# PSeitz/veloci

Measured on AMD Instinct MI355X. Metric: queries/sec, 3-term AND on 100M-doc index (p50 latency and HBM fraction alongside), higher is better.
Workload: dtype u32 doc ids + f16->f32 scores

## Files before the change

veloci_amd/csrc/scan_probe.hip:

```cpp
#include <hip/hip_runtime.h>
#include <hip/hip_fp16.h>

#include "device_types.hpp"
#include "kernel_common.hpp"
#include "kernels.hpp"
#include "probe_common.hpp"

namespace vq {

#ifdef VQ_STAMP
__device__ unsigned long long g_probe_stamp[16];
#define PS_INIT                                                      \
    unsigned long long _st0 = __builtin_amdgcn_s_memtime();          \
    const unsigned long long _t0 = _st0;                             \
    const unsigned long long _r0 = __builtin_amdgcn_s_memrealtime(); \
    unsigned long long _acc[16] = {0};
#define PS_AT(k)                                                \
    {                                                           \
        unsigned long long _st1 = __builtin_amdgcn_s_memtime(); \
        _acc[k] += _st1 - _st0;                                 \
        _st0 = _st1;                                            \
    }
#define PS_COUNT(k) _acc[k] += 1ull;
#define PS_FLUSH                                                                                             \
    _acc[14] = __builtin_amdgcn_s_memtime() - _t0;                        \
    _acc[15] = __builtin_amdgcn_s_memrealtime() - _r0;                \
    if (threadIdx.x == 0) {                                                                                  \
        _Pragma("unroll") for (int _k = 0; _k < 16; ++_k) if (_acc[_k]) atomicAdd(&g_probe_stamp[_k], _acc[_k]); \
    }
void debug_read_probe_stamps(unsigned long long* out, int reset) {
    (void)hipMemcpyFromSymbol(out, HIP_SYMBOL(g_probe_stamp), sizeof(unsigned long long) * 16);
    if (reset) {
        unsigned long long z[16] = {0};
        (void)hipMemcpyToSymbol(HIP_SYMBOL(g_probe_stamp), z, sizeof z);
    }
}
#else
#define PS_INIT
#define PS_AT(k)
#define PS_COUNT(k)
#define PS_FLUSH
#endif

constexpr uint32_t kPMaxR = 2;
constexpr uint32_t kPU = 256;
static_assert(kPU >= 256, "a round of 256 postings must fit the empty queue");
constexpr uint32_t kPR = 128;
constexpr uint32_t kPLdsShape = 8;
constexpr uint32_t kPLdsU = kPLdsShape + 24;
constexpr uint32_t kPLdsR = kPLdsU + kPU;
__host__ __device__ constexpr uint32_t probe_lds_tile(uint32_t nd) { return kPLdsR + (2 + nd) * kPR; }
__host__ __device__ constexpr uint32_t probe_lds_arr(uint32_t nd, uint32_t nb) { return probe_lds_tile(nd) + nb * (kPTW + kPRk); }
size_t scan_probe_lds_bytes(uint32_t cand_cap, uint32_t nd, uint32_t na, uint32_t arr_slot) {
    return (size_t)(probe_lds_arr(nd, nd - na) + na * arr_slot + 2 * cand_cap) * 4 + 16;
}

template <uint32_t ND, uint32_t NA, bool OR = false>
__device__ __forceinline__ void probe_body(const uint8_t* __restrict__ blob, const uint32_t span, const uint32_t q, const uint32_t cand_cap, const uint32_t arr_slot,
                                           unsigned long long* __restrict__ span_keys, unsigned long long* __restrict__ num_hits) {
    extern __shared__ __attribute__((aligned(16))) uint32_t lds[];
    const uint32_t lane = threadIdx.x;
    const VQ_CONST QHeader* H = as_const<QHeader>(blob);
    const VQ_CONST DList* gl = as_const<DList>(blob + H->off_lists);
    const VQ_CONST DOp* gops = as_const<DOp>(blob + H->off_ops);
    const VQ_CONST DProbe* P = as_const<DProbe>(blob + H->off_simple2);
    const uint32_t sflags = H->simple_flags;
    const uint32_t top_k = H->top_k;
    constexpr uint32_t n = ND + 1u;
    constexpr uint32_t NB = ND - NA;
    constexpr uint32_t NB1 = NB ? NB : 1u, NA1 = NA ? NA : 1u;
    PS_INIT

    unsigned long long* thr = reinterpret_cast<unsigned long long*>(lds);
    uint32_t* cand_n = lds + 2;
    uint32_t* sh = lds + kPLdsShape;
    uint32_t* uq = lds + kPLdsU;
    uint32_t* rq = lds + kPLdsR;
    uint32_t* tile = lds + probe_lds_tile(ND);
    uint32_t* rank = tile + NB * kPTW;
    uint32_t* arr = lds + probe_lds_arr(ND, NB);
    unsigned long long* cand = reinterpret_cast<unsigned long long*>(arr + NA * arr_slot);
    unsigned long long* const gthr = reinterpret_cast<unsigned long long*>(const_cast<uint8_t*>(blob) + offsetof(QHeader, gthr));
    CandState cs{cand, cand_n, thr, cand_cap, gthr};
    cs.upper = H->key_upper;
    uint32_t* const stat = H->stat_off ? lds + 4 : nullptr;
    uint8_t* const pool = H->off_pool ? const_cast<uint8_t*>(blob) + H->off_pool : nullptr;

    const uint32_t* ccov = nullptr;
    const uint32_t* cgdir = nullptr;
    const uint32_t* d_bitmap[NB1];
    const uint32_t* d_rank[NB1];
    const uint16_t* d_arr[NA1];
    const uint32_t* d_agd[NA1];
    {
        const uint32_t ck = (uint32_t)__ffs((int)sf_cover_mask(sflags)) - 1u;
        const uint32_t am = sf_array_mask(sflags);
        uint32_t role_of[4] = {0u, 0u, 0u, 0u};
        uint32_t ib = 0, ia = NB;
#pragma unroll
        for (uint32_t k = 0; k < n; ++k) {
            const VQ_CONST DList& d = gl[gops[k].list_begin];
            if (k == ck) {
                ccov = P->leaf[k].cov32;
                cgdir = P->leaf[k].gdir;
                if (lane == 0) {
                    sh[kShCts] = __float_as_uint(d.term_score);
                    sh[kShPrunable] = (d.term_score > 0.0f && d.max_raw < 0x7C00u) ? 1u : 0u;
                }
            } else {
                const bool is_arr = ((am >> k) & 1u) != 0u;
                const uint32_t role = is_arr ? ia : ib;
#pragma unroll
                for (uint32_t j = 0; j < NB; ++j)
                    if (!is_arr && j == role) {
                        d_bitmap[j] = d.bitmap;
                        d_rank[j] = d.rank_dir;
                    }
#pragma unroll
                for (uint32_t a = 0; a < NA; ++a)
                    if (is_arr && NB + a == role) {
                        d_arr[a] = P->leaf[k].arr16;
                        d_agd[a] = P->leaf[k].gdir;
                    }
                if (lane == 0) {
                    const uint16_t mr = d.max_raw;
                    sh[kShTs + role] = __float_as_uint(d.term_score);
                    sh[kShVmax + role] = (d.term_score > 0.0f && mr < 0x7C00u) ? __float_as_uint(posting_value(d.term_score, mr)) : 0x7F800000u;
                    reinterpret_cast<unsigned long long*>(sh + kShScores)[role] = is_arr ? (unsigned long long)(uintptr_t)P->leaf[k].cov32 : (unsigned long long)(uintptr_t)d.scores;
                }
                role_of[k] = 1u + role;
                if (is_arr) ++ia;
                else ++ib;
            }
        }
        const KOp root(gops + n);
#pragma unroll
        for (uint32_t j = 0; j < n; ++j) {
            const uint32_t k = OR ? j : root.and_order(j);
            if (lane == 0) sh[kShSrc + j] = k == 0u ? role_of[0] : k == 1u ? role_of[1] : k == 2u ? role_of[2] : role_of[3];
        }
    }

    const uint32_t n_spans = H->n_spans;
    const unsigned long long range = (unsigned long long)(H->doc_hi - H->doc_lo);
    const uint32_t span_lo = span == 0 ? H->doc_lo : ((H->doc_lo + (uint32_t)(range * span / n_spans)) & ~(kPT - 1u));
    const uint32_t span_hi = span + 1 == n_spans ? H->doc_hi : ((H->doc_lo + (uint32_t)(range * (span + 1) / n_spans)) & ~(kPT - 1u));
    const uint32_t bitmap_base = H->bitmap_base;
    const uint32_t keys_base = H->keys_base;

    if (lane == 0) {
        *thr = __hip_atomic_load(gthr, __ATOMIC_RELAXED, __HIP_MEMORY_SCOPE_AGENT);
        *cand_n = 0;
        lds[4] = 0u;
    }
    __syncthreads();
    unsigned long long thr_seen = *thr;
    uint32_t raw_min = 0u;
    constexpr uint32_t kMasks = OR ? (1u << ND) : 1u;
    uint32_t rmin[kMasks];
    auto take_raw_min = [&](const float thr_f) {
        if (OR) {
#pragma unroll
            for (uint32_t m = 0; m < kMasks; ++m) rmin[m] = probe_raw_min<ND>(sh, thr_f, lane, m);
        } else raw_min = probe_raw_min<ND>(sh, thr_f, lane);
    };
    take_raw_min(__uint_as_float(unorder_f32((uint32_t)(thr_seen >> 32))));

    const u32x4 kSent = u32x4{0xFFFFFFFFu, 0xFFFFFFFFu, 0xFFFFFFFFu, 0xFFFFFFFFu};
    const VQ_GLOBAL u32x4* cc4 = as_global(reinterpret_cast<const u32x4*>(ccov));

    uint32_t un = 0, rn = 0;
    uint32_t ucnt = 0;
    unsigned long long hits = 0;
    unsigned long long g_prev = 0ull;

    const uint32_t t_first = (span_lo - bitmap_base) >> kProbeTileShift;
    const uint32_t t_end = span_hi > span_lo ? ((span_hi - 1u - bitmap_base) >> kProbeTileShift) + 1u : t_first;
    uint32_t dir_base = t_first;
    auto load_dir = [&](const uint32_t* g) { return as_global(g)[dir_base + lane < t_end ? dir_base + lane : t_end]; };
    uint32_t dirv = load_dir(cgdir);
    uint32_t adv[NA1];
#pragma unroll
    for (uint32_t a = 0; a < NA; ++a) adv[a] = load_dir(d_agd[a]);
    auto dir_at = [&](const uint32_t v, const uint32_t tt) { return (uint32_t)__builtin_amdgcn_readlane((int)v, (int)(tt - dir_base)); };

    u32x4 wk[ND][kPNV];
    uint32_t rk[NB1];
    u32x4 nid[kPMaxR], cid[kPMaxR];
#pragma unroll
    for (uint32_t r = 0; r < kPMaxR; ++r) nid[r] = cid[r] = kSent;
    uint32_t pf_rounds = 0, pf_v0 = 0, pf_v1 = 0;
    uint32_t na_g0[NA1], na_nv[NA1];
    uint32_t a_g0[NA1], a_cnt[NA1];
#pragma unroll
    for (uint32_t a = 0; a < NA1; ++a) na_g0[a] = na_nv[a] = a_g0[a] = a_cnt[a] = 0u;
    auto issue_tile = [&](const uint32_t tt, const uint32_t g0, const uint32_t g1) {
        pf_rounds = (g1 - g0 + 31u) >> 5;
        pf_v0 = g0 * 2u;
        pf_v1 = g1 * 2u;
        if (OR || pf_rounds) {
#pragma unroll
            for (uint32_t i = 0; i < NB; ++i) {
                const VQ_GLOBAL u32x4* gb = as_global(reinterpret_cast<const u32x4*>(d_bitmap[i] + (size_t)tt * kPTW));
#pragma unroll
                for (uint32_t h = 0; h < kPNV; ++h) wk[i][h] = gb[h * 64u + lane];
                rk[i] = as_global(d_rank[i])[tt * kPRk + lane];
            }
#pragma unroll
            for (uint32_t a = 0; a < NA; ++a) {
                const VQ_GLOBAL u32x4* ga = as_global(reinterpret_cast<const u32x4*>(d_arr[a]) + na_g0[a]);
#pragma unroll
                for (uint32_t h = 0; h < kPNV; ++h)
                    if (h * 64u + lane < na_nv[a]) wk[NB + a][h] = ga[h * 64u + lane];
            }
#pragma unroll
            for (uint32_t r = 0; r < kPMaxR; ++r) {
                const uint32_t v = pf_v0 + r * 64u + lane;
                nid[r] = kSent;
                if (r < pf_rounds && v < pf_v1) nid[r] = cc4[v];
            }
        }
    };

    uint32_t tile_lo = 0;
    uint32_t f_stage = 0;
    uint32_t f_doc = 0, f_idx[ND];
    float f_vc = 0.0f, f_vd[ND];
    uint16_t f_r = 0;
    bool f_alive = false;
#pragma unroll
    for (uint32_t i = 0; i < ND; ++i) {
        f_idx[i] = 0u;
        f_vd[i] = 0.0f;
    }
    uint32_t rhead = 0;
    uint32_t tiles_since_merge = 8;
    auto push_keys = [&](const unsigned long long key, bool pending, const bool final) {
        if (wballot(pending)) {
            while (true) {
                if (pending) {
                    if (key > *thr) {
                        uint32_t pos = atomicAdd(cs.n, 1u);
                        if (pos < cs.cap) {
                            cs.cand[pos] = key;
                            pending = false;
                        }
                    } else pending = false;
                }
                probe_lds_fence();
                if (!wballot(pending)) break;
                cand_prune(cs, top_k);
            }
            if (pool && (tiles_since_merge >= 8u || final)) {
                PS_COUNT(13)
                tiles_since_merge = 0;
                probe_pool_merge<true>(cs, top_k, pool, lane);
            }
            const unsigned long long tn = *thr;
            if ((uint32_t)(tn >> 32) != (uint32_t)(thr_seen >> 32)) take_raw_min(__uint_as_float(unorder_f32((uint32_t)(tn >> 32))));
            thr_seen = tn;
        }
    };
    uint32_t f_mask = 0;
    auto sum_of = [&](const ProbeShape<ND>& S, const float vc, const float (&vd)[ND], const uint32_t mask) { return OR ? probe_or_sum<ND>(S, vc, vd, mask) : probe_sum<ND>(S, vc, vd); };
    auto flush_final = [&](const ProbeShape<ND>& S, const bool final) {
        const float score = sum_of(S, f_vc, f_vd, f_mask);
        const unsigned long long key = ((unsigned long long)order_f32(__float_as_uint(score)) << 32) | (unsigned long long)f_doc;
        f_stage = 0;
        PS_COUNT(12)
        push_keys(key, f_alive && key > *thr && key < cs.upper, final);
    };
    auto flush_service = [&](const bool final) {
        const unsigned long long* sptr = reinterpret_cast<const unsigned long long*>(sh + kShScores);
        unsigned long long gp = sptr[0];
        uint32_t gidx = 0u;
        if (f_stage) {
            const ProbeShape<ND> S = probe_shape<ND>(sh);
            const float thr_f = __uint_as_float(unorder_f32((uint32_t)(*thr >> 32)));
            bool last = true;
#pragma unroll
            for (uint32_t i = 0; i < ND; ++i)
                if (f_stage == i + 1u) {
                    f_vd[i] = posting_value(S.ts[i], f_r);
                    if (i + 1u < ND) {
                        constexpr uint32_t zero = 0;
                        f_alive = f_alive && !(sum_of(S, f_vc, f_vd, f_mask) < thr_f);
                        if (stat && lane == 0) *stat += 2u * (uint32_t)__popcll(wballot(f_alive));
                        gp = sptr[i + 1u < ND ? i + 1u : zero];
                        gidx = (f_alive && (!OR || ((f_mask >> (i + 1u < ND ? i + 1u : zero)) & 1u))) ? f_idx[i + 1u < ND ? i + 1u : zero] : 0u;
                        last = false;
                    }
                }
            if (last) flush_final(S, final);
            else ++f_stage;
        } else if (rn >= 64u || (final && rn)) {
            const uint32_t count = rn < 64u ? rn : 64u;
            probe_lds_fence();
            f_alive = lane < count;
            uint32_t raw = 0;
            const uint32_t slot = (rhead + lane) & (kPR - 1u);
            if (f_alive) {
                f_doc = rq[slot];
                raw = rq[kPR + slot];
#pragma unroll
                for (uint32_t i = 0; i < ND; ++i) f_idx[i] = rq[(2u + i) * kPR + slot];
            }
            if (OR) {
                f_mask = 0u;
#pragma unroll
                for (uint32_t i = 0; i < ND; ++i) f_mask |= f_idx[i] != 0xFFFFFFFFu ? 1u << i : 0u;
            }
            f_vc = posting_value(__uint_as_float(sh[kShCts]), (uint16_t)raw);
#pragma unroll
            for (uint32_t i = 0; i < ND; ++i) f_vd[i] = __uint_as_float(sh[kShVmax + i]);
            if (stat && lane == 0) *stat += 2u * count;
            gidx = (f_alive && (!OR || (f_mask & 1u))) ? f_idx[0] : 0u;
            f_stage = 1u;
            rhead = (rhead + count) & (kPR - 1u);
            rn -= count;
        }
        f_r = as_global(reinterpret_cast<const uint16_t*>((uintptr_t)gp))[gidx];
    };
    auto flush_sync = [&]() {
        const ProbeShape<ND> S = probe_shape<ND>(sh);
        probe_lds_fence();
        const uint32_t slot = (rhead + lane) & (kPR - 1u);
        const uint32_t doc = rq[slot];
        const float vc = posting_value(S.cts, (uint16_t)rq[kPR + slot]);
        float vd[ND];
        uint32_t mask = 0;
#pragma unroll
        for (uint32_t i = 0; i < ND; ++i) {
            const uint16_t* sp = reinterpret_cast<const uint16_t*>((uintptr_t) reinterpret_cast<const unsigned long long*>(sh + kShScores)[i]);
            const uint32_t ix = rq[(2u + i) * kPR + slot];
            if (ix != 0xFFFFFFFFu) mask |= 1u << i;
            vd[i] = posting_value(S.ts[i], as_global(sp)[(OR && ix == 0xFFFFFFFFu) ? 0u : ix]);
        }
        if (stat && lane == 0) *stat += 2u * ND * 64u;
        const float score = sum_of(S, vc, vd, mask);
        const unsigned long long key = ((unsigned long long)order_f32(__float_as_uint(score)) << 32) | (unsigned long long)doc;
        rhead = (rhead + 64u) & (kPR - 1u);
        rn -= 64u;
        push_keys(key, key > *thr && key < cs.upper, false);
    };
    auto bitmap_rank = [&](const uint32_t i, const uint32_t rel) {
        const uint32_t g = rel >> kRankShift, wi = (rel >> 5) & 15u, below = (1u << (rel & 31u)) - 1u;
        const int full = (int)((1u << wi) - 1u);
        const uint32_t* tl = tile + i * kPTW;
        uint32_t acc = rank[i * kPRk + g] + (uint32_t)__popc(tl[rel >> 5] & below);
        const u32x4* gw = reinterpret_cast<const u32x4*>(tl + g * 16u);
#pragma unroll
        for (uint32_t v4 = 0; v4 < 4; ++v4) {
            const u32x4 x = gw[v4];
            acc += (uint32_t)__popc(x.x & (uint32_t)__builtin_amdgcn_sbfe(full, v4 * 4u + 0u, 1u));
            acc += (uint32_t)__popc(x.y & (uint32_t)__builtin_amdgcn_sbfe(full, v4 * 4u + 1u, 1u));
            acc += (uint32_t)__popc(x.z & (uint32_t)__builtin_amdgcn_sbfe(full, v4 * 4u + 2u, 1u));
            acc += (uint32_t)__popc(x.w & (uint32_t)__builtin_amdgcn_sbfe(full, v4 * 4u + 3u, 1u));
        }
        return acc;
    };
    auto rank_some = [&](const uint32_t cnt) {
        while (rn + cnt > kPR) flush_sync();
        probe_lds_fence();
        const uint32_t* const uqe = uq + (un - cnt);
        un -= cnt;
        if (NA == 0u && ND == 2u && cnt <= 32u) {
            const uint32_t el = lane & 31u, role = lane >> 5;
            if (el < cnt) {
                const uint32_t e = uqe[el];
                const uint32_t rel = e >> 16;
                const uint32_t slot = (rhead + rn + el) & (kPR - 1u);
                if (role == 0u) {
                    rq[slot] = tile_lo + rel;
                    rq[kPR + slot] = e & 0xFFFFu;
                }
                const bool here = !OR || ((tile[role * kPTW + (rel >> 5)] >> (rel & 31u)) & 1u) != 0u;
                rq[(2u + role) * kPR + slot] = here ? bitmap_rank(role, rel) : 0xFFFFFFFFu;
            }
            rn += cnt;
        } else if (NA == 0u) {
            if (lane < cnt) {
                const uint32_t e = uqe[lane];
                const uint32_t rel = e >> 16;
                const uint32_t slot = (rhead + rn + lane) & (kPR - 1u);
                rq[slot] = tile_lo + rel;
                rq[kPR + slot] = e & 0xFFFFu;
#pragma unroll
                for (uint32_t i = 0; i < NB; ++i) {
                    const bool here = !OR || ((tile[i * kPTW + (rel >> 5)] >> (rel & 31u)) & 1u) != 0u;
                    rq[(2u + i) * kPR + slot] = here ? bitmap_rank(i, rel) : 0xFFFFFFFFu;
                }
            }
            rn += cnt;
        } else {
            uint32_t e = 0xFFFFFFFFu, pos[NA1];
            bool found = lane < cnt;
            if (found) e = uqe[lane];
            const uint32_t rel = e >> 16;
#pragma unroll
            for (uint32_t a = 0; a < NA; ++a) {
                const uint16_t* A = reinterpret_cast<const uint16_t*>(arr + a * arr_slot);
                uint32_t lo = 0u, len = a_cnt[a];
#ifdef VQ_PROBE_NO_SEARCH
                lo = rel & 7u;
                len = 0u;
#endif
                while (len > 1u) {
                    const uint32_t half = len >> 1;
                    lo = (uint32_t)A[lo + half] <= rel ? lo + half : lo;
                    len -= half;
                }
#ifdef VQ_PROBE_NO_SEARCH
                found = found && a_cnt[a] != 0u && ((uint32_t)A[lo] ^ rel) < 0x2000u;
#else
                found = found && a_cnt[a] != 0u && (uint32_t)A[lo] == rel;
#endif
                pos[a] = lo;
            }
            const unsigned long long fm = wballot(found);
            hits += (unsigned long long)__popcll(fm);
            const bool live = found && (e & 0xFFFFu) >= raw_min;
            const unsigned long long lm = wballot(live);
            if (lm) {
                if (live) {
                    const uint32_t slot = (rhead + rn + (uint32_t)__popcll(lm & ((1ull << lane) - 1ull))) & (kPR - 1u);
                    rq[slot] = tile_lo + rel;
                    rq[kPR + slot] = e & 0xFFFFu;
#pragma unroll
                    for (uint32_t i = 0; i < NB; ++i) rq[(2u + i) * kPR + slot] = bitmap_rank(i, rel);
#pragma unroll
                    for (uint32_t a = 0; a < NA; ++a) rq[(2u + NB + a) * kPR + slot] = (a_g0[a] * 8u + pos[a]) * 2u;
                }
                rn += (uint32_t)__popcll(lm);
            }
        }
    };
    uint32_t lo_rel = 0, width = 0;
    struct ProbeWords {
        uint32_t w[OR ? ND : 1u][4];
    };
    auto probe_read = [&](const u32x4 e4) {
        const uint32_t ee[4] = {e4.x, e4.y, e4.z, e4.w};
        ProbeWords pw;
#pragma unroll
        for (uint32_t c = 0; c < 4; ++c) {
            const uint32_t a = (ee[c] >> 21) & (kPTW - 1u);
            if (OR) {
#pragma unroll
                for (uint32_t i = 0; i < ND; ++i) pw.w[OR ? i : 0u][c] = tile[i * kPTW + a];
            } else {
                pw.w[0][c] = 0xFFFFFFFFu;
                if (NB) {
                    pw.w[0][c] = tile[a];
#pragma unroll
                    for (uint32_t i = 1; i < NB; ++i) pw.w[0][c] &= tile[i * kPTW + a];
                }
            }
        }
        return pw;
    };
    auto probe_eval = [&](const u32x4 e4, const ProbeWords& pw, const bool may_overflow) {
        const uint32_t ee[4] = {e4.x, e4.y, e4.z, e4.w};
        unsigned long long lm[4];
        bool live[4];
#pragma unroll
        for (uint32_t c = 0; c < 4; ++c) {
            const uint32_t rel = ee[c] >> 16;
            const bool in = (rel - lo_rel) < width;
            if (OR) {
                uint32_t mask = 0;
#pragma unroll
                for (uint32_t i = 0; i < ND; ++i) mask |= ((pw.w[OR ? i : 0u][c] >> (rel & 31u)) & 1u) << i;
                uint32_t need = rmin[0];
#pragma unroll
                for (uint32_t m = 1; m < kMasks; ++m) need = mask == m ? rmin[OR ? m : 0u] : need;
                hits += (unsigned long long)__popcll(wballot(in && mask == 0u));
                live[c] = in && (ee[c] & 0xFFFFu) >= need;
                lm[c] = wballot(live[c]);
                continue;
            }
            const bool bit = ((pw.w[0][c] >> (rel & 31u)) & 1u) != 0u;
            const unsigned long long sm = NB ? (wballot(in) & wballot(bit)) : wballot(in);
            if (NA == 0u) {
                const bool strong = (ee[c] & 0xFFFFu) >= raw_min;
                hits += (unsigned long long)__popcll(sm);
                lm[c] = sm & wballot(strong);
                live[c] = in && bit && strong;
            } else {
                lm[c] = sm;
                live[c] = in && bit;
            }
        }
        if (lm[0] | lm[1] | lm[2] | lm[3]) {
            if (may_overflow) {
                const uint32_t add = (uint32_t)__popcll(lm[0]) + (uint32_t)__popcll(lm[1]) + (uint32_t)__popcll(lm[2]) + (uint32_t)__popcll(lm[3]);
                while (un + add > kPU) rank_some(un < 64u ? un : 64u);
            }
#pragma unroll
            for (uint32_t c = 0; c < 4; ++c) {
                if (live[c]) uq[un + (uint32_t)__popcll(lm[c] & ((1ull << lane) - 1ull))] = ee[c];
                un += (uint32_t)__popcll(lm[c]);
            }
        }
    };

    uint32_t t = t_first;
    tile_lo = bitmap_base + (t_first << kProbeTileShift);
    auto next_arrays = [&](const uint32_t tt) {
#pragma unroll
        for (uint32_t a = 0; a < NA; ++a) {
            na_g0[a] = dir_at(adv[a], tt);
            na_nv[a] = dir_at(adv[a], tt + 1u) - na_g0[a];
        }
    };
    if (t < t_end) {
        next_arrays(t);
        issue_tile(t, dir_at(dirv, t), dir_at(dirv, t + 1u));
    }
    PS_AT(0)
    while (t < t_end) {
        PS_COUNT(8)
        __builtin_amdgcn_s_waitcnt(0x0F70);
        __builtin_amdgcn_s_setprio(3);
        const uint32_t rounds = pf_rounds, v0 = pf_v0, v1 = pf_v1;
        if (OR || rounds) {
            if (OR) {
#pragma unroll
                for (uint32_t h = 0; h < kPNV; ++h) {
                    u32x4 u = wk[0][h];
#pragma unroll
                    for (uint32_t i = 1; i < NB; ++i) u |= wk[i][h];
                    ucnt += (uint32_t)__popc(u.x) + (uint32_t)__popc(u.y) + (uint32_t)__popc(u.z) + (uint32_t)__popc(u.w);
                }
            }
#pragma unroll
            for (uint32_t i = 0; i < NB; ++i) {
#pragma unroll
                for (uint32_t h = 0; h < kPNV; ++h) reinterpret_cast<u32x4*>(tile + i * kPTW)[h * 64u + lane] = wk[i][h];
                rank[i * kPRk + lane] = rk[i];
            }
#pragma unroll
            for (uint32_t a = 0; a < NA; ++a) {
#pragma unroll
                for (uint32_t h = 0; h < kPNV; ++h)
                    if (h * 64u + lane < na_nv[a]) reinterpret_cast<u32x4*>(arr + a * arr_slot)[h * 64u + lane] = wk[NB + a][h];
                a_g0[a] = na_g0[a];
                a_cnt[a] = na_nv[a] * 8u;
            }
#pragma unroll
            for (uint32_t r = 0; r < kPMaxR; ++r) {
                cid[r] = nid[r];
                asm volatile("" : "+v"(cid[r]));
            }
        }
        {
            uint32_t fr = f_r, glo = (uint32_t)g_prev, ghi = (uint32_t)(g_prev >> 32);
            asm volatile("" : "+v"(fr), "+v"(glo), "+v"(ghi), "+v"(dirv));
#pragma unroll
            for (uint32_t a = 0; a < NA; ++a) asm volatile("" : "+v"(adv[a]));
            f_r = (uint16_t)fr;
            g_prev = ((unsigned long long)ghi << 32) | glo;
        }
        PS_AT(1)
        if (lane == 0 && g_prev > *thr) *thr = g_prev;
        const bool more = t + 1u < t_end;
        uint32_t ng0 = 0, ng1 = 0;
        if (more) {
            if (t + 2u - dir_base >= 64u) {
                dir_base = t + 1u;
                dirv = load_dir(cgdir);
#pragma unroll
                for (uint32_t a = 0; a < NA; ++a) adv[a] = load_dir(d_agd[a]);
            }
            ng0 = dir_at(dirv, t + 1u);
            ng1 = dir_at(dirv, t + 2u);
            next_arrays(t + 1u);
        }
        if (f_stage || rn >= 64u) PS_COUNT(11)
        flush_service(false);
        PS_AT(4)
        if (more) issue_tile(t + 1u, ng0, ng1);
        else pf_rounds = 0;
        if (lane == 0) g_prev = __hip_atomic_load(gthr, __ATOMIC_RELAXED, __HIP_MEMORY_SCOPE_AGENT);
        __builtin_amdgcn_s_setprio(0);
        probe_lds_fence();
        {
            const unsigned long long tn = *thr;
            if ((uint32_t)(tn >> 32) != (uint32_t)(thr_seen >> 32)) take_raw_min(__uint_as_float(unorder_f32((uint32_t)(tn >> 32))));
            thr_seen = tn;
            ++tiles_since_merge;
        }
        PS_AT(5)
#ifdef VQ_PROBE_STREAM_ONLY
        hits += (unsigned long long)__popcll(wballot((cid[0].x ^ cid[1].y) == 0x12345u));
        if (rounds && span == 0xFFFFFFFFu) {
#else
        if (rounds) {
#endif
            const uint32_t tile_end = tile_lo + kPT;
            const uint32_t tile_hi = (tile_end > tile_lo && tile_end < span_hi) ? tile_end : span_hi;
            const uint32_t lo_bound = tile_lo > span_lo ? tile_lo : span_lo;
            lo_rel = lo_bound - tile_lo;
            width = tile_hi - lo_bound;
            {
                ProbeWords pw[kPMaxR];
#pragma unroll
                for (uint32_t r = 0; r < kPMaxR; ++r)
                    if (r < rounds) pw[r] = probe_read(cid[r]);
#pragma unroll
                for (uint32_t r = 0; r < kPMaxR; ++r)
                    if (r < rounds) {
                        PS_COUNT(9)
                        probe_eval(cid[r], pw[r], r > 0u);
                    }
            }
            for (uint32_t r = kPMaxR; r < rounds; ++r) {
                const uint32_t v = v0 + r * 64u + lane;
                u32x4 e4 = kSent;
                if (v < v1) e4 = cc4[v];
                PS_COUNT(9)
                const ProbeWords pw = probe_read(e4);
                probe_eval(e4, pw, true);
            }
            PS_AT(2)
            while (un) {
                PS_COUNT(10)
                rank_some(un < 64u ? un : 64u);
            }
            PS_AT(3)
        }
        ++t;
        tile_lo += kPT;
    }
    while (f_stage || rn) flush_service(true);
    __syncthreads();
    cand_prune(cs, top_k);
    {
        const uint32_t cn = *cand_n;
        unsigned long long* out = span_keys + (size_t)keys_base + (size_t)span * top_k;
        for (uint32_t i = lane; i < top_k; i += 64u) out[i] = i < cn ? cand[i] : 0ull;
    }
    if (OR) {
        uint32_t total;
        (void)wave_excl_scan_u32(ucnt, &total);
        hits += (unsigned long long)total;
    }
    if (lane == 0 && hits) atomicAdd(&num_hits[q], hits);
    if (lane == 0 && H->stat_off && lds[4]) atomicAdd(&num_hits[H->stat_off], (unsigned long long)lds[4]);
    PS_AT(6)
    PS_FLUSH
}

__device__ __forceinline__ void probe_item(const uint32_t* __restrict__ span_base, const uint32_t* __restrict__ qmap, uint32_t nq, uint32_t* q, uint32_t* span) {
    uint32_t lo = 0, hi = nq;
    const uint32_t wg = blockIdx.x;
    while (hi - lo > 1) {
        uint32_t mid = (lo + hi) >> 1;
        if (span_base[mid] <= wg) lo = mid;
        else hi = mid;
    }
    *span = blockIdx.x - span_base[lo];
    *q = qmap[lo];
}

#define VQ_PROBE_PARAMS                                                                                                                                       \
    const uint8_t *__restrict__ blobs, const uint32_t *__restrict__ blob_off, const uint32_t *__restrict__ span_base, const uint32_t *__restrict__ qmap, uint32_t nq, \
        uint32_t cand_cap, uint32_t arr_slot, unsigned long long *__restrict__ span_keys, unsigned long long *__restrict__ num_hits
#define VQ_PROBE_ITEM                           \
    uint32_t q, span;                           \
    probe_item(span_base, qmap, nq, &q, &span); \
    const uint8_t* blob = blobs + blob_off[q];
#ifndef VQ_PROBE_WAVES
#define VQ_PROBE_WAVES 4
#endif
#define VQ_PROBE_KERNEL(waves) __global__ __launch_bounds__(64) __attribute__((amdgpu_waves_per_eu(waves, 8))) void

VQ_PROBE_KERNEL(VQ_PROBE_WAVES) k_scan_probe_1(VQ_PROBE_PARAMS) {
    VQ_PROBE_ITEM
    if (sf_array_mask(as_const<QHeader>(blob)->simple_flags) == 0u) probe_body<1, 0>(blob, span, q, cand_cap, arr_slot, span_keys, num_hits);
    else probe_body<1, 1>(blob, span, q, cand_cap, arr_slot, span_keys, num_hits);
}
VQ_PROBE_KERNEL(VQ_PROBE_WAVES) k_scan_probe_2_0(VQ_PROBE_PARAMS) {
    VQ_PROBE_ITEM
    probe_body<2, 0>(blob, span, q, cand_cap, arr_slot, span_keys, num_hits);
}
VQ_PROBE_KERNEL(VQ_PROBE_WAVES) k_scan_probe_2_1(VQ_PROBE_PARAMS) {
    VQ_PROBE_ITEM
    probe_body<2, 1>(blob, span, q, cand_cap, arr_slot, span_keys, num_hits);
}
VQ_PROBE_KERNEL(VQ_PROBE_WAVES) k_scan_probe_2_2(VQ_PROBE_PARAMS) {
    VQ_PROBE_ITEM
    probe_body<2, 2>(blob, span, q, cand_cap, arr_slot, span_keys, num_hits);
}
VQ_PROBE_KERNEL(3) k_scan_probe_3_0(VQ_PROBE_PARAMS) {
    VQ_PROBE_ITEM
    probe_body<3, 0>(blob, span, q, cand_cap, arr_slot, span_keys, num_hits);
}
VQ_PROBE_KERNEL(3) k_scan_probe_3_1(VQ_PROBE_PARAMS) {
    VQ_PROBE_ITEM
    probe_body<3, 1>(blob, span, q, cand_cap, arr_slot, span_keys, num_hits);
}
VQ_PROBE_KERNEL(3) k_scan_probe_3_2(VQ_PROBE_PARAMS) {
    VQ_PROBE_ITEM
    probe_body<3, 2>(blob, span, q, cand_cap, arr_slot, span_keys, num_hits);
}
VQ_PROBE_KERNEL(3) k_scan_probe_3_3(VQ_PROBE_PARAMS) {
    VQ_PROBE_ITEM
    probe_body<3, 3>(blob, span, q, cand_cap, arr_slot, span_keys, num_hits);
}

VQ_PROBE_KERNEL(3) k_scan_probe_or(VQ_PROBE_PARAMS) {
    VQ_PROBE_ITEM
    if (as_const<QHeader>(blob)->simple_n == 2u) probe_body<1, 0, true>(blob, span, q, cand_cap, arr_slot, span_keys, num_hits);
    else probe_body<2, 0, true>(blob, span, q, cand_cap, arr_slot, span_keys, num_hits);
}

static auto* probe_kernel(uint32_t shape) {
    return shape == kProbeAnd1 ? k_scan_probe_1 : shape == kProbeAnd2A0 ? k_scan_probe_2_0 : shape == kProbeAnd2A1 ? k_scan_probe_2_1 : shape == kProbeAnd2A2 ? k_scan_probe_2_2 :
           shape == kProbeAnd3A0 ? k_scan_probe_3_0 : shape == kProbeAnd3A1 ? k_scan_probe_3_1 : shape == kProbeAnd3A2 ? k_scan_probe_3_2 : shape == kProbeAnd3A3 ? k_scan_probe_3_3 :
                                                                                                                                                                    k_scan_probe_or;
}

uint32_t debug_probe_occupancy(uint32_t shape, size_t lds_bytes) {
    int n = 0;
    if (shape >= kProbeShapes || hipOccupancyMaxActiveBlocksPerMultiprocessor(&n, probe_kernel(shape), 64, lds_bytes) != hipSuccess || n < 0) return 0;
    return (uint32_t)n;
}

void launch_scan_probe_shape(hipStream_t st, uint32_t shape, uint32_t na_seen, uint32_t arr_slot, uint32_t total_spans, const uint8_t* blobs, const uint32_t* blob_off,
                             const uint32_t* span_base, const uint32_t* qmap, uint32_t nq, uint32_t cand_cap, unsigned long long* span_keys, unsigned long long* num_hits) {
    if (!total_spans) return;
    const uint32_t nd = shape == kProbeAnd1 ? 1u : (shape >= kProbeAnd3A0 && shape <= kProbeAnd3A3) ? 3u : 2u;
    size_t lds = 0;
    for (uint32_t na = 0; na <= nd; ++na)
        if ((na_seen >> na) & 1u) lds = std::max(lds, scan_probe_lds_bytes(cand_cap, nd, na, arr_slot));
    hipLaunchKernelGGL(probe_kernel(shape), dim3(total_spans), dim3(64), lds, st, blobs, blob_off, span_base, qmap, nq, cand_cap, arr_slot, span_keys, num_hits);
}

}
```

Measured before the change: 165,100.

## Load second candidate round slot-major to skip empty slots in AND probe

For the AND (non-OR) path, the second register round of candidate entries is now prefetched as contiguous 64-lane u32 slots instead of strided u32x4 vectors. Only the slots that hold data are evaluated, through a lighter per-slot probe that writes directly into the unranked queue. The change also guards array prefetch and store loops with wave-uniform checks and derives `live` from the ballot mask with inverse_ballot. The aim is to cut wasted LDS probes and ballots on partially filled tail rounds. It adds code-path complexity and a fallback when the queue could overflow, and the slot-major path is written only for two register rounds.

```diff
diff --git a/veloci_amd/csrc/scan_probe.hip b/veloci_amd/csrc/scan_probe.hip
--- a/veloci_amd/csrc/scan_probe.hip
+++ b/veloci_amd/csrc/scan_probe.hip
@@ -168,6 +168,8 @@
 
     const u32x4 kSent = u32x4{0xFFFFFFFFu, 0xFFFFFFFFu, 0xFFFFFFFFu, 0xFFFFFFFFu};
     const VQ_GLOBAL u32x4* cc4 = as_global(reinterpret_cast<const u32x4*>(ccov));
+    const VQ_GLOBAL uint32_t* cc1 = as_global(ccov);
+    constexpr bool kSlotMajor = !OR;
 
     uint32_t un = 0, rn = 0;
     uint32_t ucnt = 0;
@@ -211,10 +213,24 @@
                 const VQ_GLOBAL u32x4* ga = as_global(reinterpret_cast<const u32x4*>(d_arr[a]) + na_g0[a]);
 #pragma unroll
                 for (uint32_t h = 0; h < kPNV; ++h)
-                    if (h * 64u + lane < na_nv[a]) wk[NB + a][h] = ga[h * 64u + lane];
+                    if (h * 64u < na_nv[a]) {
+                        if (h * 64u + lane < na_nv[a]) wk[NB + a][h] = ga[h * 64u + lane];
+                    }
             }
 #pragma unroll
             for (uint32_t r = 0; r < kPMaxR; ++r) {
+                if (kSlotMajor && r == 1u) {
+                    const uint32_t p0 = pf_v0 * 4u + 256u, pend = pf_v1 * 4u;
+                    const VQ_GLOBAL uint32_t* cp = cc1 + p0;
+#pragma unroll
+                    for (uint32_t c = 0; c < 4; ++c)
+                        if (p0 + c * 64u < pend) {
+                            uint32_t e = 0xFFFFFFFFu;
+                            if (lane < pend - (p0 + c * 64u)) e = cp[c * 64u + lane];
+                            nid[r][c] = e;
+                        }
+                    continue;
+                }
                 const uint32_t v = pf_v0 + r * 64u + lane;
                 nid[r] = kSent;
                 if (r < pf_rounds && v < pf_v1) nid[r] = cc4[v];
@@ -439,23 +455,26 @@
     struct ProbeWords {
         uint32_t w[OR ? ND : 1u][4];
     };
+    auto and_word = [&](const uint32_t e) {
+        const uint32_t a = (e >> 21) & (kPTW - 1u);
+        uint32_t w = 0xFFFFFFFFu;
+        if (NB) {
+            w = tile[a];
+#pragma unroll
+            for (uint32_t i = 1; i < NB; ++i) w &= tile[i * kPTW + a];
+        }
+        return w;
+    };
     auto probe_read = [&](const u32x4 e4) {
         const uint32_t ee[4] = {e4.x, e4.y, e4.z, e4.w};
         ProbeWords pw;
 #pragma unroll
         for (uint32_t c = 0; c < 4; ++c) {
-            const uint32_t a = (ee[c] >> 21) & (kPTW - 1u);
             if (OR) {
+                const uint32_t a = (ee[c] >> 21) & (kPTW - 1u);
 #pragma unroll
                 for (uint32_t i = 0; i < ND; ++i) pw.w[OR ? i : 0u][c] = tile[i * kPTW + a];
-            } else {
-                pw.w[0][c] = 0xFFFFFFFFu;
-                if (NB) {
-                    pw.w[0][c] = tile[a];
-#pragma unroll
-                    for (uint32_t i = 1; i < NB; ++i) pw.w[0][c] &= tile[i * kPTW + a];
-                }
-            }
+            } else pw.w[0][c] = and_word(ee[c]);
         }
         return pw;
     };
@@ -485,11 +504,8 @@
                 const bool strong = (ee[c] & 0xFFFFu) >= raw_min;
                 hits += (unsigned long long)__popcll(sm);
                 lm[c] = sm & wballot(strong);
-                live[c] = in && bit && strong;
-            } else {
-                lm[c] = sm;
-                live[c] = in && bit;
-            }
+            } else lm[c] = sm;
+            live[c] = __builtin_amdgcn_inverse_ballot_w64(lm[c]);
         }
         if (lm[0] | lm[1] | lm[2] | lm[3]) {
             if (may_overflow) {
@@ -502,6 +518,21 @@
                 un += (uint32_t)__popcll(lm[c]);
             }
         }
+    };
+
+    auto probe_slot = [&](const uint32_t e, const uint32_t w) {
+        const uint32_t rel = e >> 16;
+        const bool in = (rel - lo_rel) < width;
+        const bool bit = ((w >> (rel & 31u)) & 1u) != 0u;
+        const unsigned long long sm = NB ? (wballot(in) & wballot(bit)) : wballot(in);
+        unsigned long long lm = sm;
+        if (NA == 0u) {
+            const bool strong = (e & 0xFFFFu) >= raw_min;
+            hits += (unsigned long long)__popcll(sm);
+            lm = sm & wballot(strong);
+        }
+        if (__builtin_amdgcn_inverse_ballot_w64(lm)) uq[un + (uint32_t)__popcll(lm & ((1ull << lane) - 1ull))] = e;
+        un += (uint32_t)__popcll(lm);
     };
 
     uint32_t t = t_first;
@@ -543,7 +574,9 @@
             for (uint32_t a = 0; a < NA; ++a) {
 #pragma unroll
                 for (uint32_t h = 0; h < kPNV; ++h)
-                    if (h * 64u + lane < na_nv[a]) reinterpret_cast<u32x4*>(arr + a * arr_slot)[h * 64u + lane] = wk[NB + a][h];
+                    if (h * 64u < na_nv[a]) {
+                        if (h * 64u + lane < na_nv[a]) reinterpret_cast<u32x4*>(arr + a * arr_slot)[h * 64u + lane] = wk[NB + a][h];
+                    }
                 a_g0[a] = na_g0[a];
                 a_cnt[a] = na_nv[a] * 8u;
             }
@@ -602,7 +635,33 @@
             const uint32_t lo_bound = tile_lo > span_lo ? tile_lo : span_lo;
             lo_rel = lo_bound - tile_lo;
             width = tile_hi - lo_bound;
-            {
+            uint32_t r_spot = kPMaxR;
+            if (kSlotMajor) {
+                static_assert(kPMaxR == 2, "the slot-major path is written for two register rounds");
+                const uint32_t behind = ((v1 - v0) * 4u - 256u + 63u) >> 6;
+                const uint32_t ns1 = behind < 4u ? behind : 4u;
+                const ProbeWords pw0 = probe_read(cid[0]);
+                uint32_t w1[2] = {0u, 0u};
+                if (rounds >= 2u) {
+                    w1[0] = and_word(cid[1].x);
+                    if (ns1 > 1u) w1[1] = and_word(cid[1].y);
+                }
+                PS_COUNT(9)
+                probe_eval(cid[0], pw0, false);
+                if (rounds >= 2u) {
+                    if (un + ns1 * 64u <= kPU) {
+                        PS_COUNT(9)
+                        probe_slot(cid[1].x, w1[0]);
+                        if (ns1 > 1u) {
+                            probe_slot(cid[1].y, w1[1]);
+                            if (ns1 > 2u) {
+                                probe_slot(cid[1].z, and_word(cid[1].z));
+                                if (ns1 > 3u) probe_slot(cid[1].w, and_word(cid[1].w));
+                            }
+                        }
+                    } else r_spot = 1u;
+                }
+            } else {
                 ProbeWords pw[kPMaxR];
 #pragma unroll
                 for (uint32_t r = 0; r < kPMaxR; ++r)
@@ -614,10 +673,16 @@
                         probe_eval(cid[r], pw[r], r > 0u);
                     }
             }
-            for (uint32_t r = kPMaxR; r < rounds; ++r) {
+            for (uint32_t r = r_spot; r < rounds; ++r) {
                 const uint32_t v = v0 + r * 64u + lane;
                 u32x4 e4 = kSent;
-                if (v < v1) e4 = cc4[v];
+                if (kSlotMajor && r < kPMaxR) {
+                    const uint32_t left = (v1 - v0) * 4u - 256u;
+                    e4.x = cid[1].x;
+                    e4.y = left > 64u ? cid[1].y : 0xFFFFFFFFu;
+                    e4.z = left > 128u ? cid[1].z : 0xFFFFFFFFu;
+                    e4.w = left > 192u ? cid[1].w : 0xFFFFFFFFu;
+                } else if (v < v1) e4 = cc4[v];
                 PS_COUNT(9)
                 const ProbeWords pw = probe_read(e4);
                 probe_eval(e4, pw, true);
```

New measurement: 166,200, median of 6. About the same (+0.6%).
